# therealadityashankar/hey-buddy

Measured on AMD Instinct MI355X. Metric: audio clips/sec featurized+trained, 1.5 s @16 kHz, 1/2/4/8 GPU, higher is better.
Workload: dtype f32

## Files before the change

### hey-buddy_amd/csrc/hbk_augment.hip

```cpp
#include <algorithm>

#include "hbk_aug_dev.h"

namespace hbk {
namespace {

static_assert(kHSlots == HBK_REVERB_SPECTRUM_SLOTS, "spectrum slot layout");
static_assert(kBsCirc == HBK_BAND_STOP_CIRCULAR_MAX_HALF && kBsPart == HBK_BAND_STOP_PARTITION_TAPS,
              "the band-stop constants of hbk.h");

struct Fft11520 {
  static constexpr int kN = kM, kLo = kTwLo;
  static constexpr bool kR16Products = true, kShortSpanWalksBlocks = true;
};
struct Fft8000 {
  static constexpr int kN = kM1, kLo = kTw8Lo;
  static constexpr bool kR16Products = false, kShortSpanWalksBlocks = false;
};

template <class F, bool INV>
__device__ __forceinline__ cf twiddle(const cf* thi, const cf* tlo, int e) {
  if constexpr ((F::kLo & (F::kLo - 1)) == 0) {
    const cf w = cmul(thi[e >> __builtin_ctz(F::kLo)], tlo[e & (F::kLo - 1)]);
    return INV ? cf{w.x, -w.y} : w;
  } else {
    const int h = e / F::kLo;
    const cf w = cmul(thi[h], tlo[e - h * F::kLo]);
    return INV ? cf{w.x, -w.y} : w;
  }
}

template <int R, bool INV>
__device__ __forceinline__ void dftr(cf (&v)[R]) {
  if constexpr (R == 16) fft16v<INV>(v);
  else if constexpr (R == 9) dft9<INV>(v);
  else if constexpr (R == 4) fft4v<INV>(v[0], v[1], v[2], v[3]);
  else dft5<INV>(v);
}

template <class F, int R, int L, int S, bool INV>
__device__ __forceinline__ void pass(cf* z, const cf* thi, const cf* tlo) {
  constexpr int kTasks = F::kN / R;
  for (int t = opaque_tid(); t < kTasks; t += kThreads) {
    constexpr int kBlocks = F::kN / (R * L);
    int blk, i;
    if constexpr (F::kShortSpanWalksBlocks && L < 16) {
      i = t / kBlocks;
      blk = t - i * kBlocks;
    } else {
      blk = t / L;
      i = t - blk * L;
    }
    cf* q = z + blk * (R * L) + i;
    cf v[R];
#pragma unroll
    for (int m = 0; m < R; ++m) v[m] = q[L * m];
    cf w[R];
    if constexpr (S != 0) {
      if constexpr (R == 16 && F::kR16Products) {
        w[1] = twiddle<F, INV>(thi, tlo, S * i);
        w[2] = twiddle<F, INV>(thi, tlo, 2 * S * i);
        w[4] = twiddle<F, INV>(thi, tlo, 4 * S * i);
        w[8] = twiddle<F, INV>(thi, tlo, 8 * S * i);
        w[3] = cmul(w[1], w[2]);
        w[5] = cmul(w[1], w[4]);
        w[6] = cmul(w[2], w[4]);
        w[7] = cmul(w[3], w[4]);
#pragma unroll
        for (int k = 9; k < 16; ++k) w[k] = cmul(w[k - 8], w[8]);
      } else {
#pragma unroll
        for (int k = 1; k < R; ++k) w[k] = twiddle<F, INV>(thi, tlo, S * i * k);
      }
    }
    if (INV && S)
#pragma unroll
      for (int k = 1; k < R; ++k) v[k] = cmul(v[k], w[k]);
    dftr<R, INV>(v);
    if (!INV && S)
#pragma unroll
      for (int k = 1; k < R; ++k) v[k] = cmul(v[k], w[k]);
#pragma unroll
    for (int m = 0; m < R; ++m) q[L * m] = v[m];
// ... 347 lines not shown
  const float* x;
  int64_t x_stride;
  float* out;
  int64_t out_stride;
  int64_t n;
  const int32_t* idx;
  const int32_t* filt;
  int n_filters;
  const float* f_lo;
  const float* f_hi;
  const int32_t* f_half;
  const int32_t* f_spec0;
  int n_spectra;
  const int32_t* s_filt;
  const int32_t* s_part;
  float2* sums;
  float* taps;
  float2* spectra;
  float* scratch;
  const float2* thi;
  const float2* tlo;
  const float2* twn;
};

__device__ __forceinline__ float bs_g(const BsLowpass& lo, const BsLowpass& hi, float2 s, int t) {
  return hi.tap(t) / s.y - lo.tap(t) / s.x;
}

__global__ void __launch_bounds__(kThreads) band_stop_sums_kernel(BandStopArgs a) {
  __shared__ float red[32];
  const int f = blockIdx.x;
  const int h = a.f_half[f];
  const BsLowpass lo(a.f_lo[f], h), hi(a.f_hi[f], h);
  double sl = 0.0, sh = 0.0;
  for (int t = static_cast<int>(threadIdx.x) - h; t <= h; t += kThreads) {
    sl += lo.tap(t);
    sh += hi.tap(t);
  }
  float fl = static_cast<float>(sl), fh = static_cast<float>(sh);
  block_sum2(fl, fh, red);
  const float2 sm = make_float2(fl, fh);
  if (threadIdx.x == 0) a.sums[f] = sm;
  if (h <= kBsCirc)
    for (int t = threadIdx.x; t <= h; t += kThreads) a.taps[int64_t(f) * (kBsCirc + 1) + t] = bs_g(lo, hi, sm, t);
}

__global__ void __launch_bounds__(kThreads) band_stop_spectrum_kernel(BandStopArgs a) {
  extern __shared__ __attribute__((aligned(16))) float smem[];
  cf* z = reinterpret_cast<cf*>(smem);
  cf* thi = reinterpret_cast<cf*>(smem + 2 * kM + 32);
  cf* tlo = thi + kTwHi;
  load_tw(thi, tlo, a.thi, a.tlo);
  const cf* twn = reinterpret_cast<const cf*>(a.twn);
  const int sidx = blockIdx.x, f = a.s_filt[sidx], p = a.s_part[sidx];
  const int h = a.f_half[f], L = 2 * h + 1;
  const BsLowpass lo(a.f_lo[f], h), hi(a.f_hi[f], h);
  const float2 sm = a.sums[f];
  for (int m = threadIdx.x; m < kT; m += kThreads) {
    float v = 0.f;
    if (p < 0) {
      const int t = m <= kT / 2 ? -m : kT - m;
      if (t >= -h && t <= h) v = bs_g(lo, hi, sm, t);
    } else {
      const int k = m == 0 ? 0 : kT - m;
      const int kk = p * kBsPart + k;
      if (k < kBsPart && kk < L) v = bs_g(lo, hi, sm, kk - h);
    }
    smem[m] = v;
  }
  __syncthreads();
  unsigned long long ph_t0 = 0;
  transform<false>(z, thi, tlo, ph_t0, 16);
  cf* H = reinterpret_cast<cf*>(a.spectra) + static_cast<int64_t>(sidx) * kHSlots;
  for (int q = threadIdx.x; q <= kM; q += kThreads) {
    const int qq = q % kM, qc = (kM - q) % kM;
    const cf zk = z[zaddr(qq)];
    const cf zc = z[zaddr(qc)];
    const cf fe = 0.5f * cf{zk.x + zc.x, zk.y - zc.y};
    const cf fo = 0.5f * cf{zk.y + zc.y, zc.x - zk.x};
    H[hslot(q)] = fe + cmul(twn[hslot(q)], fo);
  }
}

__device__ __forceinline__ void bs_multiply(cf* z, const cf* H, const cf* twn) {
  constexpr int kRest = kM / 2 / 16 + 1;
  for (int idx = opaque_tid(); idx < 16 * kRest; idx += kThreads) {
    const int c = idx / kRest;
    const int k = c + 16 * (idx - c * kRest);
    if (k > kM / 2) continue;
    const int kc = (kM - k) % kM;
    const int pz = zaddr(k);
    const cf zk = z[pz];
    const cf zc = z[zaddr(kc)];
    const cf fe = 0.5f * cf{zk.x + zc.x, zk.y - zc.y};
    const cf fo = 0.5f * cf{zk.y + zc.y, zc.x - zk.x};
    const cf wk = twn[hslot(k)];
    const cf Xk = fe + cmul(wk, fo);
    const cf Xc = cf{fe.x, -fe.y} + cmul(cf{-wk.x, wk.y}, cf{fo.x, -fo.y});
    const cf Yk = cmul(Xk, H[hslot(k)]);
    const cf Yc = cmul(Xc, H[hslot(kM - k)]);
    const cf s1 = 0.5f * cf{Yk.x + Yc.x, Yk.y - Yc.y};
    const cf d1 = 0.5f * cf{Yk.x - Yc.x, Yk.y + Yc.y};
    const cf wd = cmul(cf{wk.x, -wk.y}, d1);
    const cf s2 = 0.5f * cf{Yc.x + Yk.x, Yc.y - Yk.y};
    const cf d2 = 0.5f * cf{Yc.x - Yk.x, Yc.y + Yk.y};
    const cf wd2 = cmul(cf{-wk.x, -wk.y}, d2);
    z[pz] = s1 + cf{-wd.y, wd.x};
    if (kc != k) z[zaddr(kc)] = s2 + cf{-wd2.y, wd2.x};
  }
}

__global__ void __launch_bounds__(kThreads) band_stop_kernel(BandStopArgs a) {
  extern __shared__ __attribute__((aligned(16))) float smem[];
  cf* z = reinterpret_cast<cf*>(smem);
  cf* thi = reinterpret_cast<cf*>(smem + 2 * kM + 32);
  cf* tlo = thi + kTwHi;
  float* gt = reinterpret_cast<float*>(tlo + kTwLo);
  float* xe = gt + kBsCirc + 1;
  load_tw(thi, tlo, a.thi, a.tlo);
  const cf* twn = reinterpret_cast<const cf*>(a.twn);
  float* zf = smem;
  float* xs = a.scratch + static_cast<int64_t>(blockIdx.x) * kT;
  unsigned long long ph_t0 = 0;
  for (int64_t e = blockIdx.x; e < a.n; e += gridDim.x) {
    const int64_t clip = a.idx[e];
    const float* x = a.x + clip * a.x_stride;
    float* out = a.out + clip * a.out_stride;
    const int f = a.filt[e];
    const int h = a.f_half[f];
    const cf* H0 = reinterpret_cast<const cf*>(a.spectra) + static_cast<int64_t>(a.f_spec0[f]) * kHSlots;
    __syncthreads();
    if (h <= kBsCirc) {
      for (int s = opaque_tid(); s < kT; s += kThreads) zf[s] = x[s];
      for (int t = threadIdx.x; t <= h; t += kThreads) gt[t] = a.taps[int64_t(f) * (kBsCirc + 1) + t];
      for (int i = threadIdx.x; i < 2 * h; i += kThreads) {
        xe[i] = x[i];
        xe[2 * kBsCirc + i] = x[kT - 2 * h + i];
      }
      __syncthreads();
      const int tid = threadIdx.x;
      float corr = 0.f;
      int n_edge = -1;
      if (tid < 2 * h) {
        const float* xb = xe + 2 * kBsCirc;
        if (tid < h) {
          n_edge = tid;
          const float x0 = xe[0];
          for (int d = -h; d < -n_edge; ++d) corr += gt[-d] * (x0 - xb[2 * h + n_edge + d]);
        } else {
          n_edge = kT - 2 * h + tid;
          const float x1 = xb[2 * h - 1];
          for (int d = kT - n_edge; d <= h; ++d) corr += gt[d] * (x1 - xe[n_edge + d - kT]);
        }
      }
      transform<false>(z, thi, tlo, ph_t0, 16);
      bs_multiply(z, H0, twn);
      __syncthreads();
      transform<true>(z, thi, tlo, ph_t0, 16);
      for (int s = opaque_tid(); s < kT; s += kThreads) {
        const bool edge = s < h || s >= kT - h;
        if (!edge) out[s] = x[s] - zf[s] * (1.f / kM);
      }
      if (n_edge >= 0) {
        const float xv = n_edge < h ? xe[n_edge] : xe[2 * kBsCirc + n_edge - (kT - 2 * h)];
        out[n_edge] = xv - (zf[n_edge] * (1.f / kM) + corr);
      }
      continue;
    }
    for (int s = opaque_tid(); s < kT; s += kThreads) xs[s] = x[s];
    const int parts = (2 * h + 1 + kBsPart - 1) / kBsPart;
    for (int p = 0; p < parts; ++p) {
      const cf* Hp = H0 + static_cast<int64_t>(p) * kHSlots;
      for (int b = 0; b < 2; ++b) {
        __syncthreads();
        const int base = b * kBsHalf + p * kBsPart - h;
        for (int j = opaque_tid(); j < kT; j += kThreads) zf[j] = xs[min(max(base + j, 0), kT - 1)];
        __syncthreads();
        transform<false>(z, thi, tlo, ph_t0, 16);
        bs_multiply(z, Hp, twn);
        __syncthreads();
        transform<true>(z, thi, tlo, ph_t0, 16);
        for (int i = opaque_tid(); i < kBsHalf; i += kThreads) {
          const int n = b * kBsHalf + i;
          const float c = zf[i] * (1.f / kM);
          out[n] = (p == 0 ? xs[n] : out[n]) - c;
        }
      }
    }
  }
}

struct ColoredArgs {
  const float* x;
  int64_t x_stride;
  float* out;
  int64_t out_stride;
  int64_t n_clips;
  const float* white;
  int64_t white_stride;
  uint64_t seed;
  int64_t group;
  const float* f_decay;
  const float* snr_db;
  float lin_step;
  const int32_t* idx;
  int64_t n_entries;
  const float2* thi;
  const float2* tlo;
  const float2* twn;
  float* gbuf;
  float* grms;
  int64_t n_groups;
  int no_copy;
};

__device__ __forceinline__ uint64_t mix64(uint64_t z) {
  z = (z ^ (z >> 30)) * 0xBF58476D1CE4E5B9ull;
  z = (z ^ (z >> 27)) * 0x94D049BB133111EBull;
  return z ^ (z >> 31);
}
__device__ __forceinline__ float2 gauss2(uint64_t seed, uint64_t i) {
  const uint64_t h = mix64(seed + 0x9E3779B97F4A7C15ull * (i + 1));
  const float u1 = (static_cast<float>(h >> 40) + 0.5f) * (1.f / 16777216.f);
  const float u2 = static_cast<float>((h >> 16) & 0xFFFFFF) * (1.f / 16777216.f);
  const float r = sqrtf(-2.f * __logf(u1));
  float sn, cs;
  __sincosf(6.283185307179586f * u2, &sn, &cs);
  return make_float2(r * cs, r * sn);
}

template <bool INV>
__device__ __forceinline__ void transform8(cf* z, const cf* thi, const cf* tlo) {
  if (!INV) {
    pass<Fft8000, 16, 500, 1, false>(z, thi, tlo);
    __syncthreads();
    pass<Fft8000, 5, 100, 16, false>(z, thi, tlo);
    __syncthreads();
    pass<Fft8000, 5, 20, 80, false>(z, thi, tlo);
    __syncthreads();
    pass<Fft8000, 5, 4, 400, false>(z, thi, tlo);
    __syncthreads();
    pass<Fft8000, 4, 1, 0, false>(z, thi, tlo);
    __syncthreads();
  } else {
    pass<Fft8000, 4, 1, 0, true>(z, thi, tlo);
    __syncthreads();
    pass<Fft8000, 5, 4, 400, true>(z, thi, tlo);
    __syncthreads();
    pass<Fft8000, 5, 20, 80, true>(z, thi, tlo);
    __syncthreads();
    pass<Fft8000, 5, 100, 16, true>(z, thi, tlo);
    __syncthreads();
    pass<Fft8000, 16, 500, 1, true>(z, thi, tlo);
    __syncthreads();
  }
}

__device__ __forceinline__ int zaddr8(int f) {
  const int k1 = f & 15, r = f >> 4;
  const int k2 = r % 5, r2 = r / 5;
  const int k3 = r2 % 5, r3 = r2 / 5;
  const int k4 = r3 % 5, k5 = r3 / 5;
  return 500 * k1 + 100 * k2 + 20 * k3 + 4 * k4 + k5;
}

__device__ __forceinline__ void colored_second(const ColoredArgs& a, cf* z, const cf* thi, const cf* tlo, int tid,
                                               int64_t grp, float fd) {
  float* zf = reinterpret_cast<float*>(z);
  if (a.white) {
    const float* w = a.white + grp * a.white_stride;
    for (int s = tid; s < kN1; s += kThreads) zf[s] = w[s];
// ... 130 lines not shown
    const float snr = a.snr_db[clip];
    const int64_t grp = clip / a.group;
    float rms_g = __builtin_nanf("");
    if (snr == snr && a.f_decay[clip] == a.f_decay[grp * a.group]) rms_g = a.grms[grp];
    if (rms_g != rms_g) continue;
    const float* gb = a.gbuf + grp * kN1;
    const float* x = a.x + clip * a.x_stride;
    float ex = 0.f, en = 0.f;
#pragma unroll
    for (int u = 0; u < kPer; ++u) {
      const int s = tid + u * kThreads;
      if (s < kT) {
        const float v = *reinterpret_cast<const float*>(reinterpret_cast<const char*>(x) + (static_cast<uint32_t>(s) << 2));
        ex = fmaf(v, v, ex);
      }
    }
    block_sum2(ex, en, red);
    const float rms_x = sqrtf(ex / kT);
    const float scale = rms_x / powf(10.f, snr / 20.f) / (rms_g + 1e-8f) * (1.f / kM1);
    float* out = a.out + clip * a.out_stride;
#pragma unroll
    for (int u = 0; u < kPer; ++u) {
      const int s = tid + u * kThreads;
      if (s < kT) {
        const int sn = s < kN1 ? s : s - kN1;
        const float xv = *reinterpret_cast<const float*>(reinterpret_cast<const char*>(x) + (static_cast<uint32_t>(s) << 2));
        const float nv =
            *reinterpret_cast<const float*>(reinterpret_cast<const char*>(gb) + (static_cast<uint32_t>(sn) << 2));
        *reinterpret_cast<float*>(reinterpret_cast<char*>(out) + (static_cast<uint32_t>(s) << 2)) = fmaf(scale, nv, xv);
      }
    }
    __syncthreads();
  }
}

}

#ifdef HBK_PHASE_TIMING
int pv_phase_take(unsigned long long* out);
#endif

}

struct hbk_reverb_plan {
  void* tables = nullptr;
  const float2* thi = nullptr;
  const float2* tlo = nullptr;
  const float2* twn = nullptr;
  const float2* thi8 = nullptr;
  const float2* tlo8 = nullptr;
  const float2* twn16 = nullptr;
  hbk::SrcView view = {nullptr, 0, nullptr, nullptr};
};

extern "C" {

int hbk_reverb_plan_create(int64_t T, hbk_reverb_plan** plan) {
  using namespace hbk;
  if (!plan) return arg_error("plan is NULL");
  *plan = nullptr;
  if (T != kT) {
    set_error("hbk: reverb supports clips of %d samples (1.44 s @ 16 kHz), got %lld", kT, (long long)T);
    return HBK_ERR_UNSUPPORTED;
  }
  const ReverbTables t = reverb_tables();
  auto* p = new hbk_reverb_plan();
  hipError_t e;
  if ((e = hipMalloc(&p->tables, t.bytes())) != hipSuccess ||
      (e = hipMemcpy(p->tables, t.host.data(), t.bytes(), hipMemcpyHostToDevice)) != hipSuccess) {
    hbk_reverb_plan_destroy(p);
    return hip_error(e, "reverb plan tables");
  }
  auto table = [&](ReverbTable i) {
    return reinterpret_cast<const float2*>(static_cast<const unsigned char*>(p->tables) + t.off[i]);
  };
  p->thi = table(kTabHi), p->tlo = table(kTabLo), p->twn = table(kTabN);
  p->thi8 = table(kTabHi8), p->tlo8 = table(kTabLo8), p->twn16 = table(kTabN16);
  const struct {
    const void* kernel;
    size_t lds;
  } opt_in[] = {
      {reinterpret_cast<const void*>(augment_kernel), kAugLds},
      {reinterpret_cast<const void*>(spectrum_kernel), kAugLds},
      {reinterpret_cast<const void*>(band_stop_kernel), kBandStopLds},
      {reinterpret_cast<const void*>(band_stop_spectrum_kernel), kAugLds},
      {reinterpret_cast<const void*>(colored_noise_kernel), kColoredLds},
      {reinterpret_cast<const void*>(colored_group_kernel), kColoredLds},
  };
  for (const auto& o : opt_in)
    if ((e = hipFuncSetAttribute(o.kernel, hipFuncAttributeMaxDynamicSharedMemorySize, int(o.lds))) != hipSuccess) {
      hbk_reverb_plan_destroy(p);
      return hip_error(e, "hipFuncSetAttribute(augment LDS)");
    }
  *plan = p;
  return HBK_OK;
}

int hbk_reverb_plan_destroy(hbk_reverb_plan* p) {
  if (!p) return HBK_OK;
  (void)hipFree(p->tables);
  delete p;
  return HBK_OK;
}

int hbk_reverb_plan_set_source(hbk_reverb_plan* p, const float* src, int64_t src_stride, const int32_t* src_len,
                               const int32_t* src_pre) {
  if (!p) return hbk::arg_error("plan is NULL");
  return hbk::src_view(src, src_stride, src_len, src_pre, p->view);
}

int hbk_reverb_spectrum(const hbk_reverb_plan* p, const float* kernels, int64_t n_kernels, int64_t stride,
                        float* spectra, void* stream) {
  using namespace hbk;
  if (!p) return arg_error("plan is NULL");
  if (n_kernels < 0) return arg_error("negative n_kernels");
  if (n_kernels == 0) return HBK_OK;
  if (!kernels || !spectra) return arg_error("NULL pointer");
  if (stride < kT) return arg_error("kernel stride < 23040");
  hipLaunchKernelGGL(spectrum_kernel, dim3(unsigned(n_kernels)), dim3(kThreads), kAugLds, as_stream(stream),
                     kernels, stride, reinterpret_cast<float2*>(spectra), p->thi, p->tlo, p->twn);
  HBK_LAUNCH_CHECK("spectrum_kernel");
  return HBK_OK;
}

static int augment_args(const hbk_reverb_plan* p, const float* x, int64_t n_clips, int64_t x_stride,
                        const float* noise_ring, int64_t ring_len, const int64_t* noise_off, const float* snr_db,
                        const float* spectra, const int32_t* spec_idx, const float* gain, float* out,
                        int64_t out_stride, hbk::AugArgs& a) {
  using namespace hbk;
  if (!p) return arg_error("plan is NULL");
  if (n_clips < 0) return arg_error("negative n_clips");
  if (!x || !out || !noise_off || !snr_db || !spec_idx) return arg_error("NULL pointer");
  if (x_stride < kT || out_stride < kT) return arg_error("stride < 23040");
  if (!noise_ring && ring_len > 0) return arg_error("noise ring is NULL");
  if (ring_len >= (int64_t(1) << 30)) return arg_error("noise ring longer than 2^30 samples");
  a = AugArgs{};
  a.x = x;
  a.x_stride = x_stride;
  a.out = out;
  a.out_stride = out_stride;
  a.n_clips = n_clips;
  a.ring = noise_ring;
  a.ring_len = ring_len;
  a.noise_off = noise_off;
  a.snr_db = snr_db;
  a.spectra = reinterpret_cast<const float2*>(spectra);
  a.spec_idx = spec_idx;
  a.gain = gain;
  a.thi = p->thi;
  a.tlo = p->tlo;
  a.twn = p->twn;
  a.view = p->view;
  return HBK_OK;
}

static void augment_launch(const hbk::AugArgs& a, void* stream) {
  using namespace hbk;
  const int64_t blocks = std::min<int64_t>(a.n_clips, persistent_blocks(1, stream));
  hipLaunchKernelGGL(augment_kernel, dim3(unsigned(blocks)), dim3(kThreads), kAugLds, as_stream(stream), a);
}

int hbk_augment(const hbk_reverb_plan* p, const float* x, int64_t n_clips, int64_t x_stride,
                const float* noise_ring, int64_t ring_len, const int64_t* noise_off, const float* snr_db,
                const float* spectra, const int32_t* spec_idx, const float* gain, float* out,
                int64_t out_stride, void* stream) {
  using namespace hbk;
  if (n_clips == 0 && p) return HBK_OK;
// ... 111 lines not shown
                        float* out, int64_t out_stride, void* workspace, int64_t workspace_bytes, void* stream) {
  using namespace hbk;
  if (n_clips == 0 && p) return HBK_OK;
  AugArgs a;
  int st = augment_args(p, x, n_clips, x_stride, noise_ring, ring_len, noise_off, snr_db, spectra, spec_idx, gain,
                        out, out_stride, a);
  if (st != HBK_OK) return st;
  ColoredArgs c;
  st = colored_args(p, x, n_clips, x_stride, white, white_stride, seed, clips_per_noise, c_f_decay, c_snr_db,
                    sample_rate, c_idx, c_n_entries, out, out_stride, workspace, workspace_bytes, c);
  if (st != HBK_OK) return st;
  if (out != x && out + n_clips * out_stride > x && x + n_clips * x_stride > out)
    return arg_error("out overlaps x without being x");
  c.no_copy = 1;
  if (c.grms) {
    colored_group_launch(c, stream);
    HBK_LAUNCH_CHECK("colored_group_kernel");
  }
  if (c.n_entries > 0) {
    colored_clip_launch(c, stream);
    HBK_LAUNCH_CHECK("colored_noise_kernel");
  }
  a.c_snr = c_snr_db;
  a.c_fd = c_f_decay;
  a.c_group = clips_per_noise;
  a.c_gbuf = c.gbuf;
  a.c_grms = c.grms;
  augment_launch(a, stream);
  HBK_LAUNCH_CHECK("augment_kernel");
  return HBK_OK;
}

int64_t hbk_band_stop_workspace_size(int64_t n, int32_t n_filters, int32_t n_spectra, void* stream) {
  using namespace hbk;
  if (n <= 0) return 0;
  return band_stop_layout(n, n_filters, n_spectra, std::min<int64_t>(n, persistent_blocks(1, stream))).total;
}

int hbk_band_stop(const hbk_reverb_plan* p, const float* x, int64_t x_stride, int64_t n, const int32_t* idx,
                  const int32_t* filt, int32_t n_filters, const float* f_lo, const float* f_hi,
                  const int32_t* f_half, const int32_t* f_spec0, int32_t n_spectra, const int32_t* s_filt,
                  const int32_t* s_part, float* out, int64_t out_stride, void* workspace, int64_t workspace_bytes,
                  void* stream) {
  using namespace hbk;
  if (!p) return arg_error("plan is NULL");
  if (n < 0 || n_filters < 0 || n_spectra < 0) return arg_error("negative count");
  if (n == 0) return HBK_OK;
  if (n_filters == 0 || n_spectra < n_filters) return arg_error("every filter needs at least one spectrum");
  if (!x || !idx || !filt || !f_lo || !f_hi || !f_half || !f_spec0 || !s_filt || !s_part || !out || !workspace)
    return arg_error("NULL pointer");
  if (x_stride < kT || out_stride < kT) return arg_error("stride < 23040");
  const int64_t blocks = std::min<int64_t>(n, persistent_blocks(1, stream));
  const BandStopLayout off = band_stop_layout(n, n_filters, n_spectra, blocks);
  if (workspace_bytes < off.total) return arg_error("workspace too small (hbk_band_stop_workspace_size)");
  BandStopArgs a;
  a.x = x;
  a.x_stride = x_stride;
  a.out = out;
  a.out_stride = out_stride;
  a.n = n;
  a.idx = idx;
  a.filt = filt;
  a.n_filters = n_filters;
  a.f_lo = f_lo;
  a.f_hi = f_hi;
  a.f_half = f_half;
  a.f_spec0 = f_spec0;
  a.n_spectra = n_spectra;
  a.s_filt = s_filt;
  a.s_part = s_part;
  unsigned char* w = static_cast<unsigned char*>(workspace);
  a.sums = reinterpret_cast<float2*>(w + off.sums);
  a.taps = reinterpret_cast<float*>(w + off.taps);
  a.spectra = reinterpret_cast<float2*>(w + off.spectra);
  a.scratch = reinterpret_cast<float*>(w + off.scratch);
  a.thi = p->thi;
  a.tlo = p->tlo;
  a.twn = p->twn;
  hipStream_t st = as_stream(stream);
  hipLaunchKernelGGL(band_stop_sums_kernel, dim3(unsigned(n_filters)), dim3(kThreads), 0, st, a);
  HBK_LAUNCH_CHECK("band_stop_sums_kernel");
  hipLaunchKernelGGL(band_stop_spectrum_kernel, dim3(unsigned(n_spectra)), dim3(kThreads), kAugLds, st, a);
  HBK_LAUNCH_CHECK("band_stop_spectrum_kernel");
  hipLaunchKernelGGL(band_stop_kernel, dim3(unsigned(blocks)), dim3(kThreads), kBandStopLds, st, a);
  HBK_LAUNCH_CHECK("band_stop_kernel");
  return HBK_OK;
}

}

#ifdef HBK_PHASE_TIMING
extern "C" int hbk_debug_aug_phase(unsigned long long* out) {
  if (hipMemcpyFromSymbol(out, HIP_SYMBOL(hbk::g_aug_phase), sizeof(unsigned long long) * 32) != hipSuccess)
    return -2;
  unsigned long long z[32] = {};
  (void)hipMemcpyToSymbol(HIP_SYMBOL(hbk::g_aug_phase), z, sizeof(z));
  unsigned long long pv[5];
  if (hbk::pv_phase_take(pv) != 0) return -2;
  for (int i = 0; i < 5; ++i) out[16 + i] += pv[i];
  return 0;
}
#endif
```

### hey-buddy_amd/csrc/hbk_clip_ops.hip

```cpp
#include <algorithm>

#include "hbk_aug_dev.h"

namespace hbk {
namespace {

struct TanhArgs {
  const float* x;
  int64_t x_stride;
  float* out;
  int64_t out_stride;
  int64_t n_clips;
  const float* amount;
  const int32_t* idx;
  int64_t n_entries;
  SrcView view;
};

__device__ __forceinline__ unsigned abs_bits(float v, int s) {
  return s < kT ? (__builtin_bit_cast(unsigned, v) & 0x7FFFFFFFu) : 0xFFFFFFFFu;
}

__global__ void __launch_bounds__(kThreads) __attribute__((amdgpu_waves_per_eu(8)))
tanh_distortion_kernel(TanhArgs a) {
  __shared__ unsigned hist[4096];
  __shared__ float red[32];
  __shared__ unsigned pick[2];
  constexpr int kPer = (kT + kThreads - 1) / kThreads;
  const int64_t n_iter = a.idx ? a.n_entries : a.n_clips;
  for (int64_t e = blockIdx.x; e < n_iter; e += gridDim.x) {
    const int64_t clip = a.idx ? a.idx[e] : e;
    const int tid = opaque_tid();
    const float* x = a.x + clip * a.x_stride;
    float* out = a.out + clip * a.out_stride;
    const float amt = a.amount[clip];
    if (amt != amt) {
      if (out != x) copy_clip(x, out, tid);
      continue;
    }
    float xr[kPer];
    const int pre = a.view.pre ? a.view.pre[clip] : -1, len = a.view.pre ? a.view.len[clip] : 0;
    if (pre >= 0) {
      const int n = min(len, kT);
      const float* row = n > 0 ? a.view.src + clip * a.view.stride : x;
      const int t = opaque_tid();
      const int w0 = __builtin_amdgcn_readfirstlane(t & ~63);
#pragma unroll
      for (int u = 0; u < kPer; ++u) xr[u] = load_placed_wave(row, pre, n, w0 + u * kThreads, t & 63);
    } else {
    const int t = opaque_tid();
#pragma unroll
    for (int u = 0; u < kPer; ++u) {
      const int s = t + u * kThreads;
      xr[u] = s < kT ? *reinterpret_cast<const float*>(reinterpret_cast<const char*>(x) + (static_cast<uint32_t>(s) << 2))
                     : 0.f;
    }
    }
    const double pos = (100.0 - 99.0 * static_cast<double>(amt)) / 100.0 * (kT - 1);
    const int lo = min(max(static_cast<int>(floor(pos)), 0), kT - 1);
    const double frac = pos - lo;
    unsigned prefix = 0, mask = 0, rank = static_cast<unsigned>(lo);
#pragma unroll 1
    for (int p = 0; p < 3; ++p) {
      const int shift = p == 0 ? 19 : (p == 1 ? 9 : 0), bins = p == 0 ? 4096 : (p == 1 ? 1024 : 512);
      const int per_lane = bins >> 6;
      for (int i = tid; i < bins; i += kThreads) hist[i] = 0;
      __syncthreads();
      const int t = opaque_tid();
#pragma unroll
      for (int u = 0; u < kPer; ++u) {
        const unsigned b = abs_bits(xr[u], t + u * kThreads);
        if ((b & mask) == prefix && b != 0xFFFFFFFFu) atomicAdd(&hist[(b >> shift) & (bins - 1)], 1u);
      }
      __syncthreads();
      if (tid < 64) {
        unsigned own = 0;
        for (int i = 0; i < per_lane; ++i) own += hist[per_lane * tid + i];
        unsigned inc = own;
#pragma unroll
        for (int d = 1; d < 64; d <<= 1) {
          const unsigned v = __shfl_up(inc, d, 64);
          if (tid >= d) inc += v;
        }
        const unsigned long long hit = __ballot(inc > rank);
        const int l = __ffsll(static_cast<long long>(hit)) - 1;
        if (tid == l) {
          unsigned r = rank - (inc - own), dsel = per_lane * l;
          for (int i = 0; i < per_lane - 1; ++i) {
            const unsigned h = hist[dsel];
            if (r < h) break;
            r -= h;
            ++dsel;
          }
          pick[0] = dsel;
          pick[1] = r;
        }
      }
      __syncthreads();
      prefix |= pick[0] << shift;
      mask |= static_cast<unsigned>(bins - 1) << shift;
      rank = pick[1];
    }
    float cnt = 0.f, mg = __builtin_inff();
    const int t2 = opaque_tid();
#pragma unroll
    for (int u = 0; u < kPer; ++u) {
      const unsigned b = abs_bits(xr[u], t2 + u * kThreads);
      if (b == 0xFFFFFFFFu) continue;
      if (b <= prefix) cnt += 1.f;
      else mg = fminf(mg, __builtin_bit_cast(float, b));
    }
    cnt = block_sum(cnt, red);
    {
      for (int d = 32; d >= 1; d >>= 1) mg = fminf(mg, __shfl_xor(mg, d, 64));
      __syncthreads();
      if ((tid & 63) == 0) red[tid >> 6] = mg;
      __syncthreads();
      mg = red[0];
      for (int w = 1; w < kThreads / 64; ++w) mg = fminf(mg, red[w]);
    }
    const double v_lo = __builtin_bit_cast(float, prefix);
    const double v_hi = (cnt >= lo + 2 || lo + 1 >= kT) ? v_lo : static_cast<double>(mg);
    const double d = v_hi - v_lo;
    const double th = frac >= 0.5 ? v_hi - d * (1.0 - frac) : v_lo + d * frac;
    const float g = static_cast<float>(0.5 / (th + 1e-6));
    float ex = 0.f, ey = 0.f;
#pragma unroll
    for (int u = 0; u < kPer; ++u) {
      ex += xr[u] * xr[u];
      xr[u] = 1.f - __fdividef(2.f, __expf(2.f * g * xr[u]) + 1.f);
      ey += xr[u] * xr[u];
    }
    block_sum2(ex, ey, red);
    const float rms_x = sqrtf(ex / kT);
    const float post = rms_x > 1e-9f ? rms_x / sqrtf(ey / kT) : 1.f;
    const int t3 = opaque_tid();
#pragma unroll
    for (int u = 0; u < kPer; ++u) {
      const int s = t3 + u * kThreads;
      if (s < kT) *reinterpret_cast<float*>(reinterpret_cast<char*>(out) + (static_cast<uint32_t>(s) << 2)) = xr[u] * post;
    }
    __syncthreads();
  }
}

constexpr int kPlaceSpan = 4096;
__global__ void __launch_bounds__(256) place_kernel(const float* __restrict__ src, int64_t src_stride,
                                                    const int32_t* __restrict__ src_len,
                                                    const int32_t* __restrict__ pre,
                                                    const int32_t* __restrict__ idx, float* __restrict__ out,
                                                    int64_t out_stride, int64_t n_clips, int T) {
  const int spans = (T + kPlaceSpan - 1) / kPlaceSpan;
  const int64_t items = n_clips * spans;
  constexpr int kR = kPlaceSpan / 1024;
  for (int64_t it = blockIdx.x; it < items; it += gridDim.x) {
    const int64_t e = it / spans;
    const int sp = static_cast<int>(it - e * spans);
    const int64_t clip = idx ? idx[e] : e;
    const int p = pre[clip];
    const int n = min(src_len[clip], T);
    const int last = max(n - 1, 0);
    const float* s = src + clip * src_stride;
    float* o = out + clip * out_stride;
    const int t0 = sp * kPlaceSpan + 4 * static_cast<int>(threadIdx.x);
    float v[kR][4];
#pragma unroll
    for (int r = 0; r < kR; ++r)
#pragma unroll
      for (int q = 0; q < 4; ++q) {
        const int u = t0 + r * 1024 + q - p;
        const float x = n > 0 ? s[min(max(u, 0), last)] : 0.f;
        v[r][q] = (u >= 0 && u < n) ? x : 0.f;
      }
#pragma unroll
    for (int r = 0; r < kR; ++r) {
      const int t = t0 + r * 1024;
      if (t < T) *reinterpret_cast<float4*>(o + t) = make_float4(v[r][0], v[r][1], v[r][2], v[r][3]);
    }
  }
}

constexpr int kEqTile = 64;
struct EqArgs {
  const float* x;
  int64_t x_stride;
  const double* coef;
  const int32_t* idx;
  float* out;
  int64_t out_stride;
  int64_t n;
  SrcView view;
};

constexpr int kEqClips = 8;
__global__ void __launch_bounds__(64) eq_kernel(EqArgs a) {
  constexpr int kRow = kEqTile + 4;
  __shared__ __attribute__((aligned(16))) float tin[kEqClips][kRow];
  __shared__ __attribute__((aligned(16))) float tout[kEqClips][kRow];
  const int lane = threadIdx.x, c = lane >> 3, sec = lane & 7;
  const int64_t j0 = static_cast<int64_t>(blockIdx.x) * kEqClips;
  const int64_t jc = min(j0 + c, a.n - 1);
  const double* cf0 = a.coef + jc * 35;
  const bool copy = cf0[0] != cf0[0];
  const int k = min(sec, 6);
  double b0 = cf0[5 * k], b1 = cf0[5 * k + 1], b2 = cf0[5 * k + 2], a1 = cf0[5 * k + 3], a2 = cf0[5 * k + 4];
  if (copy) b0 = 1.0, b1 = b2 = a1 = a2 = 0.0;
  double s1 = 0.0, s2 = 0.0;
  const int lc = lane >> 3, lq = lane & 7;
  const int64_t jl = min(j0 + lc, a.n - 1);
  const int64_t clip_l = a.idx ? static_cast<int64_t>(a.idx[jl]) : jl;
  const float* xl = a.x + clip_l * a.x_stride;
  float* ol = a.out + clip_l * a.out_stride;
  const bool store_l = j0 + lc < a.n;
  const int pre_l = a.view.pre ? a.view.pre[clip_l] : -1, len_l = a.view.pre ? a.view.len[clip_l] : 0;
  const int n_l = pre_l >= 0 ? min(len_l, kT) : 0;
  const float* sl = n_l > 0 ? a.view.src + clip_l * a.view.stride : xl;
  float4 p0, p1;
  auto load_tile = [&](int t) {
    const int u0 = t + 4 * lq - pre_l;
    if (pre_l >= 0 && u0 >= 0 && u0 + 35 < n_l) {
      const float* q = sl + u0;
      p0 = float4{q[0], q[1], q[2], q[3]};
      p1 = float4{q[32], q[33], q[34], q[35]};
// ... 32 lines not shown
#pragma unroll
      for (int q = 0; q < 8; ++q) {
        const float u = sec == 0 ? in8[q] : prev;
        const double vd = u;
        const double y = fma(b0, vd, s1);
        s1 = fma(b1, vd, fma(-a1, y, s2));
        s2 = fma(b2, vd, -a2 * y);
        const float v = static_cast<float>(y);
        o8[q] = v;
        prev = __builtin_bit_cast(float, __builtin_amdgcn_update_dpp(__builtin_bit_cast(int, prev),
                                                                     __builtin_bit_cast(int, v), 0x111, 0xF, 0xF,
                                                                     false));
      }
      if (sec == 6) {
        *reinterpret_cast<float4*>(&tout[c][st0]) = float4{o8[0], o8[1], o8[2], o8[3]};
        *reinterpret_cast<float4*>(&tout[c][st0 + 4]) = float4{o8[4], o8[5], o8[6], o8[7]};
      }
    }
    __syncthreads();
    if (store_l) {
#pragma unroll
      for (int m = 0; m < 8; ++m) {
        const int kk = lq + 8 * m;
        const int n = t0 - 6 + kk;
        if (n >= 0 && n < kT) ol[n] = tout[lc][kk];
      }
    }
    __syncthreads();
  }
}

}
}

extern "C" {

int hbk_place_clips_idx(const float* src, int64_t n_clips, int64_t src_stride, const int32_t* src_len,
                        const int32_t* pre, const int32_t* idx, int64_t n_entries, float* out, int64_t out_stride,
                        int64_t T, void* stream) {
  using namespace hbk;
  if (n_clips < 0 || (idx && n_entries < 0)) return arg_error("negative count");
  const int64_t n_rows = idx ? n_entries : n_clips;
  if (n_rows == 0) return HBK_OK;
  if (!src || !src_len || !pre || !out) return arg_error("NULL pointer");
  if (T <= 0 || T % 4 || T > (int64_t(1) << 30)) return arg_error("T must be a positive multiple of 4");
  if (out_stride < T || out_stride % 4 || (reinterpret_cast<uintptr_t>(out) & 15))
    return arg_error("out rows must be 16-B aligned with stride >= T");
  const int64_t items = n_rows * ((T + kPlaceSpan - 1) / kPlaceSpan);
  if (items >= (int64_t(1) << 31)) return arg_error("too many clips for one launch");
  const int64_t blocks = items;
  hipLaunchKernelGGL(place_kernel, dim3(unsigned(blocks)), dim3(256), 0, as_stream(stream), src, src_stride, src_len,
                     pre, idx, out, out_stride, n_rows, int(T));
  HBK_LAUNCH_CHECK("place_kernel");
  return HBK_OK;
}

int hbk_place_clips(const float* src, int64_t n_clips, int64_t src_stride, const int32_t* src_len,
                    const int32_t* pre, float* out, int64_t out_stride, int64_t T, void* stream) {
  return hbk_place_clips_idx(src, n_clips, src_stride, src_len, pre, nullptr, 0, out, out_stride, T, stream);
}

int hbk_tanh_distortion_src(const float* x, int64_t n_clips, int64_t x_stride, const float* amount,
                            const int32_t* idx, int64_t n_entries, float* out, int64_t out_stride,
                            const float* src, int64_t src_stride, const int32_t* src_len, const int32_t* src_pre,
                            void* stream) {
  using namespace hbk;
  if (n_clips < 0) return arg_error("negative n_clips");
  if (n_clips == 0) return HBK_OK;
  if (!x || !out || !amount) return arg_error("NULL pointer");
  if (x_stride < kT || out_stride < kT) return arg_error("stride < 23040");
  TanhArgs a;
  a.x = x;
  a.x_stride = x_stride;
  a.out = out;
  a.out_stride = out_stride;
  a.n_clips = n_clips;
  a.amount = amount;
  a.idx = idx;
  a.n_entries = idx ? n_entries : n_clips;
  const int st = src_view(src, src_stride, src_len, src_pre, a.view);
  if (st != HBK_OK) return st;
  if (a.n_entries <= 0) return n_entries < 0 ? arg_error("negative n_entries") : HBK_OK;
  const int64_t blocks = std::min<int64_t>(a.n_entries, persistent_blocks(2, stream));
  hipLaunchKernelGGL(tanh_distortion_kernel, dim3(unsigned(blocks)), dim3(kThreads), 0, as_stream(stream), a);
  HBK_LAUNCH_CHECK("tanh_distortion_kernel");
  return HBK_OK;
}

int hbk_tanh_distortion(const float* x, int64_t n_clips, int64_t x_stride, const float* amount,
                        const int32_t* idx, int64_t n_entries, float* out, int64_t out_stride, void* stream) {
  return hbk_tanh_distortion_src(x, n_clips, x_stride, amount, idx, n_entries, out, out_stride, nullptr, 0, nullptr,
                                 nullptr, stream);
}

int hbk_seven_band_eq_src(const float* x, int64_t n_clips, int64_t x_stride, const double* coef, const int32_t* idx,
                          int64_t n_entries, float* out, int64_t out_stride, const float* src, int64_t src_stride,
                          const int32_t* src_len, const int32_t* src_pre, void* stream) {
  using namespace hbk;
  if (n_clips < 0 || n_entries < 0) return arg_error("negative count");
  if (!idx) n_entries = n_clips;
  if (n_entries == 0) return HBK_OK;
  if (!x || !out || !coef) return arg_error("NULL pointer");
  if (x_stride < kT || out_stride < kT) return arg_error("stride < 23040");
  if ((reinterpret_cast<uintptr_t>(x) | reinterpret_cast<uintptr_t>(out)) % 16 || x_stride % 4 || out_stride % 4)
    return arg_error("x / out rows must be 16-B aligned");
  EqArgs a;
  a.x = x;
  a.x_stride = x_stride;
  a.coef = coef;
  a.idx = idx;
  a.out = out;
  a.out_stride = out_stride;
  a.n = n_entries;
  const int st = src_view(src, src_stride, src_len, src_pre, a.view);
  if (st != HBK_OK) return st;
  hipLaunchKernelGGL(eq_kernel, dim3(unsigned((n_entries + kEqClips - 1) / kEqClips)), dim3(64), 0,
                     as_stream(stream), a);
  HBK_LAUNCH_CHECK("eq_kernel");
  return HBK_OK;
}

int hbk_seven_band_eq(const float* x, int64_t n_clips, int64_t x_stride, const double* coef, const int32_t* idx,
                      int64_t n_entries, float* out, int64_t out_stride, void* stream) {
  return hbk_seven_band_eq_src(x, n_clips, x_stride, coef, idx, n_entries, out, out_stride, nullptr, 0, nullptr,
                               nullptr, stream);
}

}
```

Before: 1.130 million.

## Prefetch next clip into registers in band-stop and tanh persistent kernels

```diff
diff --git a/hey-buddy_amd/csrc/hbk_augment.hip b/hey-buddy_amd/csrc/hbk_augment.hip
--- a/hey-buddy_amd/csrc/hbk_augment.hip
+++ b/hey-buddy_amd/csrc/hbk_augment.hip
@@ -1,4 +1,5 @@
 #include <algorithm>
+#include <cstdlib>
 
 #include "hbk_aug_dev.h"
 
@@ -512,23 +513,40 @@
   }
 }
 
+template <bool kBatch>
 __device__ __forceinline__ void bs_multiply(cf* z, const cf* H, const cf* twn) {
   constexpr int kRest = kM / 2 / 16 + 1;
-  for (int idx = opaque_tid(); idx < 16 * kRest; idx += kThreads) {
+  constexpr int kIt = (16 * kRest + kThreads - 1) / kThreads;
+  const int ts = opaque_tid();
+  cf hk[kIt], hc[kIt], wn[kIt];
+  if (kBatch) {
+#pragma unroll
+    for (int it = 0; it < kIt; ++it) {
+      const int idx = min(ts + it * kThreads, 16 * kRest - 1);
+      const int c = idx / kRest;
+      const int k = min(c + 16 * (idx - c * kRest), kM / 2);
+      hk[it] = H[hslot(k)];
+      hc[it] = H[hslot(kM - k)];
+      wn[it] = twn[hslot(k)];
+    }
+  }
+#pragma unroll
+  for (int it = 0; it < kIt; ++it) {
+    const int idx = ts + it * kThreads;
     const int c = idx / kRest;
     const int k = c + 16 * (idx - c * kRest);
-    if (k > kM / 2) continue;
+    if (idx >= 16 * kRest || k > kM / 2) continue;
     const int kc = (kM - k) % kM;
     const int pz = zaddr(k);
     const cf zk = z[pz];
     const cf zc = z[zaddr(kc)];
     const cf fe = 0.5f * cf{zk.x + zc.x, zk.y - zc.y};
     const cf fo = 0.5f * cf{zk.y + zc.y, zc.x - zk.x};
-    const cf wk = twn[hslot(k)];
+    const cf wk = kBatch ? wn[it] : twn[hslot(k)];
     const cf Xk = fe + cmul(wk, fo);
     const cf Xc = cf{fe.x, -fe.y} + cmul(cf{-wk.x, wk.y}, cf{fo.x, -fo.y});
-    const cf Yk = cmul(Xk, H[hslot(k)]);
-    const cf Yc = cmul(Xc, H[hslot(kM - k)]);
+    const cf Yk = cmul(Xk, kBatch ? hk[it] : H[hslot(k)]);
+    const cf Yc = cmul(Xc, kBatch ? hc[it] : H[hslot(kM - k)]);
     const cf s1 = 0.5f * cf{Yk.x + Yc.x, Yk.y - Yc.y};
     const cf d1 = 0.5f * cf{Yk.x - Yc.x, Yk.y + Yc.y};
     const cf wd = cmul(cf{wk.x, -wk.y}, d1);
@@ -540,6 +558,7 @@
   }
 }
 
+template <bool kPipe>
 __global__ void __launch_bounds__(kThreads) band_stop_kernel(BandStopArgs a) {
   extern __shared__ __attribute__((aligned(16))) float smem[];
   cf* z = reinterpret_cast<cf*>(smem);
@@ -552,20 +571,57 @@
   float* zf = smem;
   float* xs = a.scratch + static_cast<int64_t>(blockIdx.x) * kT;
   unsigned long long ph_t0 = 0;
+  constexpr int kPer = (kT + kThreads - 1) / kThreads;
+  float xr[kPer];
+  auto prefetch = [&](int64_t clip) {
+    const float* x = a.x + clip * a.x_stride;
+    const int t = opaque_tid();
+#pragma unroll
+    for (int u = 0; u < kPer; ++u)
+      xr[u] = *reinterpret_cast<const float*>(reinterpret_cast<const char*>(x) +
+                                              (static_cast<uint32_t>(min(t + u * kThreads, kT - 1)) << 2));
+  };
+  int clip_w = 0, f_w = 0, h_w = 0;
+  if (kPipe && blockIdx.x < a.n) {
+    clip_w = a.idx[blockIdx.x];
+    f_w = a.filt[blockIdx.x];
+    h_w = a.f_half[f_w];
+    prefetch(clip_w);
+  }
   for (int64_t e = blockIdx.x; e < a.n; e += gridDim.x) {
-    const int64_t clip = a.idx[e];
+    const int64_t clip = kPipe ? clip_w : a.idx[e];
     const float* x = a.x + clip * a.x_stride;
     float* out = a.out + clip * a.out_stride;
-    const int f = a.filt[e];
-    const int h = a.f_half[f];
+    const int f = kPipe ? f_w : a.filt[e];
+    const int h = kPipe ? h_w : a.f_half[f];
+    const bool next = kPipe && e + gridDim.x < a.n;
+    if (next) {
+      clip_w = __builtin_amdgcn_readfirstlane(a.idx[e + gridDim.x]);
+      f_w = __builtin_amdgcn_readfirstlane(a.filt[e + gridDim.x]);
+      h_w = __builtin_amdgcn_readfirstlane(a.f_half[f_w]);
+    }
+    const int64_t clip_next = clip_w;
     const cf* H0 = reinterpret_cast<const cf*>(a.spectra) + static_cast<int64_t>(a.f_spec0[f]) * kHSlots;
     __syncthreads();
     if (h <= kBsCirc) {
-      for (int s = opaque_tid(); s < kT; s += kThreads) zf[s] = x[s];
-      for (int t = threadIdx.x; t <= h; t += kThreads) gt[t] = a.taps[int64_t(f) * (kBsCirc + 1) + t];
-      for (int i = threadIdx.x; i < 2 * h; i += kThreads) {
-        xe[i] = x[i];
-        xe[2 * kBsCirc + i] = x[kT - 2 * h + i];
+      if (kPipe) {
+        for (int t = threadIdx.x; t <= h; t += kThreads) gt[t] = a.taps[int64_t(f) * (kBsCirc + 1) + t];
+        const int t = opaque_tid();
+#pragma unroll
+        for (int u = 0; u < kPer; ++u) {
+          const int s = t + u * kThreads;
+          if (s < kT) zf[s] = xr[u];
+          if (u == 0 && s < 2 * h) xe[s] = xr[u];
+          if ((u + 1) * kThreads > kT - 2 * kBsCirc && s >= kT - 2 * h && s < kT)
+            xe[2 * kBsCirc + s - (kT - 2 * h)] = xr[u];
+        }
+      } else {
+        for (int s = opaque_tid(); s < kT; s += kThreads) zf[s] = x[s];
+        for (int t = threadIdx.x; t <= h; t += kThreads) gt[t] = a.taps[int64_t(f) * (kBsCirc + 1) + t];
+        for (int i = threadIdx.x; i < 2 * h; i += kThreads) {
+          xe[i] = x[i];
+          xe[2 * kBsCirc + i] = x[kT - 2 * h + i];
+        }
       }
       __syncthreads();
       const int tid = threadIdx.x;
@@ -584,12 +640,25 @@
         }
       }
       transform<false>(z, thi, tlo, ph_t0, 16);
-      bs_multiply(z, H0, twn);
+      bs_multiply<kPipe>(z, H0, twn);
       __syncthreads();
       transform<true>(z, thi, tlo, ph_t0, 16);
-      for (int s = opaque_tid(); s < kT; s += kThreads) {
-        const bool edge = s < h || s >= kT - h;
-        if (!edge) out[s] = x[s] - zf[s] * (1.f / kM);
+      if (kPipe) {
+        const int t = opaque_tid();
+        float d[kPer];
+#pragma unroll
+        for (int u = 0; u < kPer; ++u) d[u] = xr[u] - zf[min(t + u * kThreads, kT - 1)] * (1.f / kM);
+        if (next) prefetch(clip_next);
+#pragma unroll
+        for (int u = 0; u < kPer; ++u) {
+          const int s = t + u * kThreads;
+          if (s < kT && !(s < h || s >= kT - h)) out[s] = d[u];
+        }
+      } else {
+        for (int s = opaque_tid(); s < kT; s += kThreads) {
+          const bool edge = s < h || s >= kT - h;
+          if (!edge) out[s] = x[s] - zf[s] * (1.f / kM);
+        }
       }
       if (n_edge >= 0) {
         const float xv = n_edge < h ? xe[n_edge] : xe[2 * kBsCirc + n_edge - (kT - 2 * h)];
@@ -597,7 +666,14 @@
       }
       continue;
     }
-    for (int s = opaque_tid(); s < kT; s += kThreads) xs[s] = x[s];
+    if (kPipe) {
+      const int t = opaque_tid();
+#pragma unroll
+      for (int u = 0; u < kPer; ++u)
+        if (t + u * kThreads < kT) xs[t + u * kThreads] = xr[u];
+    } else {
+      for (int s = opaque_tid(); s < kT; s += kThreads) xs[s] = x[s];
+    }
     const int parts = (2 * h + 1 + kBsPart - 1) / kBsPart;
     for (int p = 0; p < parts; ++p) {
       const cf* Hp = H0 + static_cast<int64_t>(p) * kHSlots;
@@ -607,7 +683,7 @@
         for (int j = opaque_tid(); j < kT; j += kThreads) zf[j] = xs[min(max(base + j, 0), kT - 1)];
         __syncthreads();
         transform<false>(z, thi, tlo, ph_t0, 16);
-        bs_multiply(z, Hp, twn);
+        bs_multiply<kPipe>(z, Hp, twn);
         __syncthreads();
         transform<true>(z, thi, tlo, ph_t0, 16);
         for (int i = opaque_tid(); i < kBsHalf; i += kThreads) {
@@ -617,6 +693,7 @@
         }
       }
     }
+    if (next) prefetch(clip_next);
   }
 }
 
@@ -913,7 +990,8 @@
   } opt_in[] = {
       {reinterpret_cast<const void*>(augment_kernel), kAugLds},
       {reinterpret_cast<const void*>(spectrum_kernel), kAugLds},
-      {reinterpret_cast<const void*>(band_stop_kernel), kBandStopLds},
+      {reinterpret_cast<const void*>(band_stop_kernel<false>), kBandStopLds},
+      {reinterpret_cast<const void*>(band_stop_kernel<true>), kBandStopLds},
       {reinterpret_cast<const void*>(band_stop_spectrum_kernel), kAugLds},
       {reinterpret_cast<const void*>(colored_noise_kernel), kColoredLds},
       {reinterpret_cast<const void*>(colored_group_kernel), kColoredLds},
@@ -1191,7 +1269,9 @@
   HBK_LAUNCH_CHECK("band_stop_sums_kernel");
   hipLaunchKernelGGL(band_stop_spectrum_kernel, dim3(unsigned(n_spectra)), dim3(kThreads), kAugLds, st, a);
   HBK_LAUNCH_CHECK("band_stop_spectrum_kernel");
-  hipLaunchKernelGGL(band_stop_kernel, dim3(unsigned(blocks)), dim3(kThreads), kBandStopLds, st, a);
+  const char* form = getenv("HBK_BAND_STOP_FORM");
+  hipLaunchKernelGGL(form && form[0] == '0' ? band_stop_kernel<false> : band_stop_kernel<true>, dim3(unsigned(blocks)),
+                     dim3(kThreads), kBandStopLds, st, a);
   HBK_LAUNCH_CHECK("band_stop_kernel");
   return HBK_OK;
 }
diff --git a/hey-buddy_amd/csrc/hbk_clip_ops.hip b/hey-buddy_amd/csrc/hbk_clip_ops.hip
--- a/hey-buddy_amd/csrc/hbk_clip_ops.hip
+++ b/hey-buddy_amd/csrc/hbk_clip_ops.hip
@@ -1,4 +1,5 @@
 #include <algorithm>
+#include <cstdlib>
 
 #include "hbk_aug_dev.h"
 
@@ -21,6 +22,7 @@
   return s < kT ? (__builtin_bit_cast(unsigned, v) & 0x7FFFFFFFu) : 0xFFFFFFFFu;
 }
 
+template <bool kPipe>
 __global__ void __launch_bounds__(kThreads) __attribute__((amdgpu_waves_per_eu(8)))
 tanh_distortion_kernel(TanhArgs a) {
   __shared__ unsigned hist[4096];
@@ -28,34 +30,62 @@
   __shared__ unsigned pick[2];
   constexpr int kPer = (kT + kThreads - 1) / kThreads;
   const int64_t n_iter = a.idx ? a.n_entries : a.n_clips;
+  struct Ctl {
+    int64_t clip;
+    float amt;
+    int pre, len;
+  };
+  auto ctl = [&](int64_t e) {
+    Ctl c;
+    c.clip = a.idx ? a.idx[e] : e;
+    c.amt = a.amount[c.clip];
+    c.pre = a.view.pre ? a.view.pre[c.clip] : -1;
+    c.len = a.view.pre ? a.view.len[c.clip] : 0;
+    return c;
+  };
+  auto load_clip = [&](float (&xr)[kPer], const Ctl& c) {
+    const float* x = a.x + c.clip * a.x_stride;
+    if (c.pre >= 0) {
+      const int n = min(c.len, kT);
+      const float* row = n > 0 ? a.view.src + c.clip * a.view.stride : x;
+      const int t = opaque_tid();
+      const int w0 = __builtin_amdgcn_readfirstlane(t & ~63);
+#pragma unroll
+      for (int u = 0; u < kPer; ++u) xr[u] = load_placed_wave(row, c.pre, n, w0 + u * kThreads, t & 63);
+    } else {
+      const int t = opaque_tid();
+#pragma unroll
+      for (int u = 0; u < kPer; ++u) {
+        const int s = t + u * kThreads;
+        xr[u] = s < kT ? *reinterpret_cast<const float*>(reinterpret_cast<const char*>(x) + (static_cast<uint32_t>(s) << 2))
+                       : 0.f;
+      }
+    }
+  };
+  float xr[kPer];
+  Ctl cur{}, nxt{};
+  if (kPipe && blockIdx.x < n_iter) {
+    cur = ctl(blockIdx.x);
+    if (cur.amt == cur.amt) load_clip(xr, cur);
+  }
   for (int64_t e = blockIdx.x; e < n_iter; e += gridDim.x) {
-    const int64_t clip = a.idx ? a.idx[e] : e;
+    if (!kPipe) cur = ctl(e);
+    const bool next = kPipe && e + gridDim.x < n_iter;
+    if (next) nxt = ctl(e + gridDim.x);
+    const int64_t clip = cur.clip;
     const int tid = opaque_tid();
     const float* x = a.x + clip * a.x_stride;
     float* out = a.out + clip * a.out_stride;
-    const float amt = a.amount[clip];
+    const float amt = cur.amt;
     if (amt != amt) {
       if (out != x) copy_clip(x, out, tid);
+      if (next) {
+        if (nxt.amt == nxt.amt) load_clip(xr, nxt);
+        cur = nxt;
+      }
       continue;
     }
-    float xr[kPer];
-    const int pre = a.view.pre ? a.view.pre[clip] : -1, len = a.view.pre ? a.view.len[clip] : 0;
-    if (pre >= 0) {
-      const int n = min(len, kT);
-      const float* row = n > 0 ? a.view.src + clip * a.view.stride : x;
-      const int t = opaque_tid();
-      const int w0 = __builtin_amdgcn_readfirstlane(t & ~63);
-#pragma unroll
-      for (int u = 0; u < kPer; ++u) xr[u] = load_placed_wave(row, pre, n, w0 + u * kThreads, t & 63);
-    } else {
-    const int t = opaque_tid();
-#pragma unroll
-    for (int u = 0; u < kPer; ++u) {
-      const int s = t + u * kThreads;
-      xr[u] = s < kT ? *reinterpret_cast<const float*>(reinterpret_cast<const char*>(x) + (static_cast<uint32_t>(s) << 2))
-                     : 0.f;
-    }
-    }
+    if (!kPipe) load_clip(xr, cur);
     const double pos = (100.0 - 99.0 * static_cast<double>(amt)) / 100.0 * (kT - 1);
     const int lo = min(max(static_cast<int>(floor(pos)), 0), kT - 1);
     const double frac = pos - lo;
@@ -67,11 +97,15 @@
       for (int i = tid; i < bins; i += kThreads) hist[i] = 0;
       __syncthreads();
       const int t = opaque_tid();
+      unsigned zeros = 0;
 #pragma unroll
       for (int u = 0; u < kPer; ++u) {
         const unsigned b = abs_bits(xr[u], t + u * kThreads);
-        if ((b & mask) == prefix && b != 0xFFFFFFFFu) atomicAdd(&hist[(b >> shift) & (bins - 1)], 1u);
-      }
+        if (kPipe) zeros += __popcll(__ballot(b == 0u));
+        if ((!kPipe || b != 0u) && (b & mask) == prefix && b != 0xFFFFFFFFu)
+          atomicAdd(&hist[(b >> shift) & (bins - 1)], 1u);
+      }
+      if (kPipe && prefix == 0u && zeros != 0u && (t & 63) == 0) atomicAdd(&hist[0], zeros);
       __syncthreads();
       if (tid < 64) {
         unsigned own = 0;
@@ -127,9 +161,9 @@
     float ex = 0.f, ey = 0.f;
 #pragma unroll
     for (int u = 0; u < kPer; ++u) {
-      ex += xr[u] * xr[u];
+      ex = fmaf(xr[u], xr[u], ex);
       xr[u] = 1.f - __fdividef(2.f, __expf(2.f * g * xr[u]) + 1.f);
-      ey += xr[u] * xr[u];
+      ey = fmaf(xr[u], xr[u], ey);
     }
     block_sum2(ex, ey, red);
     const float rms_x = sqrtf(ex / kT);
@@ -139,6 +173,10 @@
     for (int u = 0; u < kPer; ++u) {
       const int s = t3 + u * kThreads;
       if (s < kT) *reinterpret_cast<float*>(reinterpret_cast<char*>(out) + (static_cast<uint32_t>(s) << 2)) = xr[u] * post;
+    }
+    if (next) {
+      if (nxt.amt == nxt.amt) load_clip(xr, nxt);
+      cur = nxt;
     }
     __syncthreads();
   }
@@ -337,7 +375,9 @@
   if (st != HBK_OK) return st;
   if (a.n_entries <= 0) return n_entries < 0 ? arg_error("negative n_entries") : HBK_OK;
   const int64_t blocks = std::min<int64_t>(a.n_entries, persistent_blocks(2, stream));
-  hipLaunchKernelGGL(tanh_distortion_kernel, dim3(unsigned(blocks)), dim3(kThreads), 0, as_stream(stream), a);
+  const char* form = getenv("HBK_TANH_FORM");
+  hipLaunchKernelGGL(form && form[0] == '0' ? tanh_distortion_kernel<false> : tanh_distortion_kernel<true>,
+                     dim3(unsigned(blocks)), dim3(kThreads), 0, as_stream(stream), a);
   HBK_LAUNCH_CHECK("tanh_distortion_kernel");
   return HBK_OK;
 }
```

New measurement: 1.133 million (median of 2 runs). Within noise of the previous version (+0.3%).
